# svip-lab/impersonator

Hardware: NVIDIA H100
Metric: frames/sec @256x256 (per-frame inference hot path) (higher is better)
Workload: dtype f16 main product + e4m3 correction products (hi/lo split), f32 accumulate

## Files before the change

### impersonator_b200/csrc/common.cuh

```cuda
#pragma once
#include <cuda_runtime.h>
#include <cuda_fp16.h>
#include <stdint.h>
#include <stdio.h>

#include "../../include/lwb_b200.h"

namespace lwb {

void set_error(const char* fmt, ...);

#define LWB_CHECK_ARG(cond, msg)                                                   \
    do { if (!(cond)) { lwb::set_error("%s: %s", __func__, msg); return LWB_E_INVALID; } } while (0)

#define LWB_CUDA_OK(expr)                                                          \
    do { cudaError_t e__ = (expr); if (e__ != cudaSuccess) {                       \
        lwb::set_error("%s: %s -> %s", __func__, #expr, cudaGetErrorString(e__));  \
        return LWB_E_CUDA; } } while (0)

#define LWB_LAUNCH_OK()                                                            \
    do { cudaError_t e__ = cudaGetLastError(); if (e__ != cudaSuccess) {           \
        lwb::set_error("%s: launch failed -> %s", __func__, cudaGetErrorString(e__)); \
        return LWB_E_CUDA; } } while (0)

static inline int ceil_div(long a, long b) { return (int)((a + b - 1) / b); }

int sm_count();
constexpr int kMaxDevices = 64;
int device_slot();

bool pdl_enabled();
__device__ __forceinline__ void pdl_wait() { asm volatile("griddepcontrol.wait;" ::: "memory"); }
__device__ __forceinline__ void pdl_trigger() { asm volatile("griddepcontrol.launch_dependents;" ::: "memory"); }

template <typename... KArgs, typename... Args>
static inline cudaError_t launch_pdl(void (*kernel)(KArgs...), dim3 grid, dim3 block, size_t smem, cudaStream_t st, Args&&... args)
{
    cudaLaunchConfig_t cfg = {};
    cfg.gridDim = grid; cfg.blockDim = block; cfg.dynamicSmemBytes = smem; cfg.stream = st;
    cudaLaunchAttribute at[1];
    at[0].id = cudaLaunchAttributeProgrammaticStreamSerialization;
    at[0].val.programmaticStreamSerializationAllowed = 1;
    cfg.attrs = at; cfg.numAttrs = pdl_enabled() ? 1 : 0;
    return cudaLaunchKernelEx(&cfg, kernel, static_cast<KArgs>(args)...);
}

__device__ __forceinline__ void ldg_f32x8(const float* p, float* v) {
    const float4 a = __ldg(reinterpret_cast<const float4*>(p)), b = __ldg(reinterpret_cast<const float4*>(p) + 1);
    v[0] = a.x; v[1] = a.y; v[2] = a.z; v[3] = a.w; v[4] = b.x; v[5] = b.y; v[6] = b.z; v[7] = b.w;
}
__device__ __forceinline__ void stg_f32x8(float* p, const float* v) {
    reinterpret_cast<float4*>(p)[0] = make_float4(v[0], v[1], v[2], v[3]);
    reinterpret_cast<float4*>(p)[1] = make_float4(v[4], v[5], v[6], v[7]);
}

}
```

### impersonator_b200/csrc/conv_tc.cu

```cuda
#include <cuda.h>

#include <stdlib.h>

#include <algorithm>
#include <new>
#include <type_traits>

#include "common.cuh"

namespace {

constexpr int TILE_H = 16, TILE_W = 8;
constexpr int SWAP_N_TILE = 64;
constexpr int SWAP_TILE_H = 32;
constexpr int KCHUNK = 64;
constexpr int ROW_BYTES = TILE_W * 128;
constexpr int MAX_TAPS = 49;
constexpr int MAX_GROUP = 8;
constexpr int RING_BYTES = 200 * 1024;
constexpr int MAX_STAGES = 8;
constexpr int NUM_CONSUMERS = 256;
constexpr int NUM_THREADS = NUM_CONSUMERS + 128;
constexpr int MAX_N_TILE = 128;
static_assert(2 * 2 * (TILE_H + MAX_GROUP - 1) * ROW_BYTES + 2 * 2 * MAX_N_TILE * 128 <= RING_BYTES,
// ... 29 lines not shown
struct Cfg {
    static constexpr int B_BYTES = N_TILE * 128;
    static constexpr int B_STAGE_BYTES = B_BYTES * (SPLIT ? 2 : 1);
    static constexpr int BAR_BYTES = 4 * MAX_STAGES * 8;
    static constexpr int STATS_PARTS = N_TILE < SWAP_N_TILE ? 8 : N_TILE == SWAP_N_TILE ? 2 : 0;
    static constexpr int STATS_BYTES = STATS_PARTS * N_TILE * 8;
    static constexpr int SMEM_BYTES = 1024 + RING_BYTES + BAR_BYTES + STATS_BYTES;
    static_assert(B_STAGE_BYTES % 1024 == 0, "B entries must keep the 1024-byte swizzle alignment");
    static_assert(SMEM_BYTES <= 227 * 1024, "exceeds the shared memory of a block");
};

__device__ __forceinline__ uint32_t smem_u32(const void* p) { return (uint32_t)__cvta_generic_to_shared(p); }

__device__ __forceinline__ void mbar_init(uint64_t* bar, uint32_t count) {
    asm volatile("mbarrier.init.shared::cta.b64 [%0], %1;" ::"r"(smem_u32(bar)), "r"(count));
}
__device__ __forceinline__ void mbar_expect_tx(uint64_t* bar, uint32_t bytes) {
    asm volatile("mbarrier.arrive.expect_tx.shared::cta.b64 _, [%0], %1;" ::"r"(smem_u32(bar)), "r"(bytes) : "memory");
}
__device__ __forceinline__ void mbar_arrive(uint64_t* bar) {
    asm volatile("mbarrier.arrive.shared::cta.b64 _, [%0];" ::"r"(smem_u32(bar)) : "memory");
}
__device__ __forceinline__ bool mbar_try_wait(uint64_t* bar, uint32_t parity) {
    uint32_t ok;
    asm volatile("{\n\t.reg .pred p;\n\t"
                 "mbarrier.try_wait.parity.shared::cta.b64 p, [%1], %2;\n\t"
                 "selp.u32 %0, 1, 0, p;\n\t}"
                 : "=r"(ok) : "r"(smem_u32(bar)), "r"(parity) : "memory");
    return ok != 0;
}
__device__ __forceinline__ void mbar_wait(uint64_t* bar, uint32_t parity) {
    if (mbar_try_wait(bar, parity)) return;
    const long long t0 = clock64();
    while (!mbar_try_wait(bar, parity)) {
        if (clock64() - t0 > 4000000000ll) __trap();
    }
}
__device__ __forceinline__ bool elect_one() {
    uint32_t pred;
    asm volatile("{\n\t.reg .pred P;\n\telect.sync _|P, 0xffffffff;\n\tselp.b32 %0, 1, 0, P;\n\t}" : "=r"(pred));
    return pred != 0;
}
__device__ __forceinline__ void fence_barrier_init() { asm volatile("fence.mbarrier_init.release.cluster;" ::: "memory"); }
__device__ __forceinline__ void fence_proxy_async() { asm volatile("fence.proxy.async.shared::cta;" ::: "memory"); }

__device__ __forceinline__ void tma_load_4d(const CUtensorMap* map, void* dst, uint64_t* bar, int c0, int c1, int c2, int c3) {
    asm volatile("cp.async.bulk.tensor.4d.shared::cluster.global.mbarrier::complete_tx::bytes [%0], [%1, {%3, %4, %5, %6}], [%2];"
                 :: "r"(smem_u32(dst)), "l"(map), "r"(smem_u32(bar)), "r"(c0), "r"(c1), "r"(c2), "r"(c3) : "memory");
}
__device__ __forceinline__ void tma_load_3d(const CUtensorMap* map, void* dst, uint64_t* bar, int c0, int c1, int c2) {
    asm volatile("cp.async.bulk.tensor.3d.shared::cluster.global.mbarrier::complete_tx::bytes [%0], [%1, {%3, %4, %5}], [%2];"
                 :: "r"(smem_u32(dst)), "l"(map), "r"(smem_u32(bar)), "r"(c0), "r"(c1), "r"(c2) : "memory");
}

__device__ __forceinline__ uint64_t make_desc(uint32_t smem_addr) {
    return (uint64_t)((smem_addr & 0x3FFFF) >> 4) | (1ull << 16) | (64ull << 32) | (1ull << 62);
}
__device__ __forceinline__ void wgmma_fence() { asm volatile("wgmma.fence.sync.aligned;" ::: "memory"); }
__device__ __forceinline__ void wgmma_commit() { asm volatile("wgmma.commit_group.sync.aligned;" ::: "memory"); }
template <int N>
__device__ __forceinline__ void wgmma_wait() { asm volatile("wgmma.wait_group.sync.aligned %0;" :: "n"(N) : "memory"); }
__device__ __forceinline__ void acc_fence(float& r) { asm volatile("" : "+f"(r) :: "memory"); }

template <int N> __device__ __forceinline__ void wgmma_f16(float* d, uint64_t da, uint64_t db);
template <int N> __device__ __forceinline__ void wgmma_e4m3(float* d, uint64_t da, uint64_t db);
template <> __device__ __forceinline__ void wgmma_f16<16>(float* d, uint64_t da, uint64_t db) {
    asm volatile("{\n\t.reg .pred p;\n\tsetp.ne.b32 p, %10, 0;\n\t"
                 "wgmma.mma_async.sync.aligned.m64n16k16.f32.f16.f16 {%0, %1, %2, %3, %4, %5, %6, %7}, %8, %9, p, 1, 1, 0, 0;\n\t}"
                 : "+f"(d[0]), "+f"(d[1]), "+f"(d[2]), "+f"(d[3]), "+f"(d[4]), "+f"(d[5]), "+f"(d[6]), "+f"(d[7])
                 : "l"(da), "l"(db), "r"(1));
}
template <> __device__ __forceinline__ void wgmma_f16<32>(float* d, uint64_t da, uint64_t db) {
    asm volatile("{\n\t.reg .pred p;\n\tsetp.ne.b32 p, %18, 0;\n\t"
                 "wgmma.mma_async.sync.aligned.m64n32k16.f32.f16.f16 {%0, %1, %2, %3, %4, %5, %6, %7, %8, %9, %10, %11, %12, %13, %14, %15}, %16, %17, p, 1, 1, 0, 0;\n\t}"
                 : "+f"(d[0]), "+f"(d[1]), "+f"(d[2]), "+f"(d[3]), "+f"(d[4]), "+f"(d[5]), "+f"(d[6]), "+f"(d[7]), "+f"(d[8]), "+f"(d[9]), "+f"(d[10]), "+f"(d[11]), "+f"(d[12]), "+f"(d[13]), "+f"(d[14]), "+f"(d[15])
                 : "l"(da), "l"(db), "r"(1));
}
template <> __device__ __forceinline__ void wgmma_f16<128>(float* d, uint64_t da, uint64_t db) {
    asm volatile("{\n\t.reg .pred p;\n\tsetp.ne.b32 p, %66, 0;\n\t"
                 "wgmma.mma_async.sync.aligned.m64n128k16.f32.f16.f16 {%0, %1, %2, %3, %4, %5, %6, %7, %8, %9, %10, %11, %12, %13, %14, %15, %16, %17, %18, %19, %20, %21, %22, %23, %24, %25, %26, %27, %28, %29, %30, %31, %32, %33, %34, %35, %36, %37, %38, %39, %40, %41, %42, %43, %44, %45, %46, %47, %48, %49, %50, %51, %52, %53, %54, %55, %56, %57, %58, %59, %60, %61, %62, %63}, %64, %65, p, 1, 1, 0, 0;\n\t}"
                 : "+f"(d[0]), "+f"(d[1]), "+f"(d[2]), "+f"(d[3]), "+f"(d[4]), "+f"(d[5]), "+f"(d[6]), "+f"(d[7]), "+f"(d[8]), "+f"(d[9]), "+f"(d[10]), "+f"(d[11]), "+f"(d[12]), "+f"(d[13]), "+f"(d[14]), "+f"(d[15]), "+f"(d[16]), "+f"(d[17]), "+f"(d[18]), "+f"(d[19]), "+f"(d[20]), "+f"(d[21]), "+f"(d[22]), "+f"(d[23]), "+f"(d[24]), "+f"(d[25]), "+f"(d[26]), "+f"(d[27]), "+f"(d[28]), "+f"(d[29]), "+f"(d[30]), "+f"(d[31]), "+f"(d[32]), "+f"(d[33]), "+f"(d[34]), "+f"(d[35]), "+f"(d[36]), "+f"(d[37]), "+f"(d[38]), "+f"(d[39]), "+f"(d[40]), "+f"(d[41]), "+f"(d[42]), "+f"(d[43]), "+f"(d[44]), "+f"(d[45]), "+f"(d[46]), "+f"(d[47]), "+f"(d[48]), "+f"(d[49]), "+f"(d[50]), "+f"(d[51]), "+f"(d[52]), "+f"(d[53]), "+f"(d[54]), "+f"(d[55]), "+f"(d[56]), "+f"(d[57]), "+f"(d[58]), "+f"(d[59]), "+f"(d[60]), "+f"(d[61]), "+f"(d[62]), "+f"(d[63])
                 : "l"(da), "l"(db), "r"(1));
}
template <> __device__ __forceinline__ void wgmma_e4m3<16>(float* d, uint64_t da, uint64_t db) {
    asm volatile("{\n\t.reg .pred p;\n\tsetp.ne.b32 p, %10, 0;\n\t"
                 "wgmma.mma_async.sync.aligned.m64n16k32.f32.e4m3.e4m3 {%0, %1, %2, %3, %4, %5, %6, %7}, %8, %9, p, 1, 1;\n\t}"
                 : "+f"(d[0]), "+f"(d[1]), "+f"(d[2]), "+f"(d[3]), "+f"(d[4]), "+f"(d[5]), "+f"(d[6]), "+f"(d[7])
                 : "l"(da), "l"(db), "r"(1));
}
template <> __device__ __forceinline__ void wgmma_e4m3<32>(float* d, uint64_t da, uint64_t db) {
    asm volatile("{\n\t.reg .pred p;\n\tsetp.ne.b32 p, %18, 0;\n\t"
                 "wgmma.mma_async.sync.aligned.m64n32k32.f32.e4m3.e4m3 {%0, %1, %2, %3, %4, %5, %6, %7, %8, %9, %10, %11, %12, %13, %14, %15}, %16, %17, p, 1, 1;\n\t}"
                 : "+f"(d[0]), "+f"(d[1]), "+f"(d[2]), "+f"(d[3]), "+f"(d[4]), "+f"(d[5]), "+f"(d[6]), "+f"(d[7]), "+f"(d[8]), "+f"(d[9]), "+f"(d[10]), "+f"(d[11]), "+f"(d[12]), "+f"(d[13]), "+f"(d[14]), "+f"(d[15])
                 : "l"(da), "l"(db), "r"(1));
}
template <> __device__ __forceinline__ void wgmma_e4m3<128>(float* d, uint64_t da, uint64_t db) {
    asm volatile("{\n\t.reg .pred p;\n\tsetp.ne.b32 p, %66, 0;\n\t"
                 "wgmma.mma_async.sync.aligned.m64n128k32.f32.e4m3.e4m3 {%0, %1, %2, %3, %4, %5, %6, %7, %8, %9, %10, %11, %12, %13, %14, %15, %16, %17, %18, %19, %20, %21, %22, %23, %24, %25, %26, %27, %28, %29, %30, %31, %32, %33, %34, %35, %36, %37, %38, %39, %40, %41, %42, %43, %44, %45, %46, %47, %48, %49, %50, %51, %52, %53, %54, %55, %56, %57, %58, %59, %60, %61, %62, %63}, %64, %65, p, 1, 1;\n\t}"
                 : "+f"(d[0]), "+f"(d[1]), "+f"(d[2]), "+f"(d[3]), "+f"(d[4]), "+f"(d[5]), "+f"(d[6]), "+f"(d[7]), "+f"(d[8]), "+f"(d[9]), "+f"(d[10]), "+f"(d[11]), "+f"(d[12]), "+f"(d[13]), "+f"(d[14]), "+f"(d[15]), "+f"(d[16]), "+f"(d[17]), "+f"(d[18]), "+f"(d[19]), "+f"(d[20]), "+f"(d[21]), "+f"(d[22]), "+f"(d[23]), "+f"(d[24]), "+f"(d[25]), "+f"(d[26]), "+f"(d[27]), "+f"(d[28]), "+f"(d[29]), "+f"(d[30]), "+f"(d[31]), "+f"(d[32]), "+f"(d[33]), "+f"(d[34]), "+f"(d[35]), "+f"(d[36]), "+f"(d[37]), "+f"(d[38]), "+f"(d[39]), "+f"(d[40]), "+f"(d[41]), "+f"(d[42]), "+f"(d[43]), "+f"(d[44]), "+f"(d[45]), "+f"(d[46]), "+f"(d[47]), "+f"(d[48]), "+f"(d[49]), "+f"(d[50]), "+f"(d[51]), "+f"(d[52]), "+f"(d[53]), "+f"(d[54]), "+f"(d[55]), "+f"(d[56]), "+f"(d[57]), "+f"(d[58]), "+f"(d[59]), "+f"(d[60]), "+f"(d[61]), "+f"(d[62]), "+f"(d[63])
                 : "l"(da), "l"(db), "r"(1));
}

__device__ __forceinline__ void consumer_sync() { asm volatile("bar.sync 1, 256;" ::: "memory"); }

struct TileCoord {
    int n_idx, img, y0, x0;
};
template <int TH>
__device__ __forceinline__ TileCoord decode_tile(const ConvParams& P, int tile, int m_tiles) {
    TileCoord t;
    t.n_idx = tile / m_tiles;
    const int m_idx = tile % m_tiles;
    t.img = m_idx / (P.tiles_y * P.tiles_x);
    const int rem = m_idx % (P.tiles_y * P.tiles_x);
    t.y0 = (rem / P.tiles_x) * TH; t.x0 = (rem % P.tiles_x) * TILE_W;
    return t;
}

template <int N_TILE>
__device__ __forceinline__ void warp_tile_stats(const float* acc, bool v0, bool v1, int warp, unsigned lane, float2* s_stats)
{
#pragma unroll
    for (int j = 0; j < N_TILE / 8; j++) {
        const float a0 = v0 ? acc[4 * j] : 0.f, a1 = v0 ? acc[4 * j + 1] : 0.f;
        const float b0 = v1 ? acc[4 * j + 2] : 0.f, b1 = v1 ? acc[4 * j + 3] : 0.f;
        float s0 = a0 + b0, s1 = a1 + b1, q0 = a0 * a0 + b0 * b0, q1 = a1 * a1 + b1 * b1;
#pragma unroll
        for (int off = 4; off <= 16; off <<= 1) {
            s0 += __shfl_xor_sync(0xffffffffu, s0, off); s1 += __shfl_xor_sync(0xffffffffu, s1, off);
            q0 += __shfl_xor_sync(0xffffffffu, q0, off); q1 += __shfl_xor_sync(0xffffffffu, q1, off);
        }
        if (lane < 4) {
            s_stats[warp * N_TILE + 8 * j + 2 * lane] = make_float2(s0, q0);
            s_stats[warp * N_TILE + 8 * j + 2 * lane + 1] = make_float2(s1, q1);
        }
    }
}

template <int N_TILE, int PARTS>
__device__ __forceinline__ void flush_tile_stats(const ConvParams& P, const float2* s_stats, int img, int n_idx)
{
    consumer_sync();
    for (int col = threadIdx.x; col < N_TILE; col += NUM_CONSUMERS) {
        float s = 0.f, q = 0.f;
#pragma unroll
        for (int w = 0; w < PARTS; w++) { const float2 v = s_stats[w * N_TILE + col]; s += v.x; q += v.y; }
        int ch = n_idx * N_TILE + col;
        if (P.phase_cols > 0) ch %= P.phase_cols;
        double* dst = P.stats + 2 * ((size_t)img * P.cout + ch);
        atomicAdd(dst, (double)s);
        atomicAdd(dst + 1, (double)q);
    }
    consumer_sync();
}

template <int N_TILE>
__device__ __forceinline__ void epilogue_plain(const ConvParams& P, float* acc, const TileCoord& t, int warp, unsigned lane,
// ... 74 lines not shown
#pragma unroll
                for (int h = 0; h < 2; h++) {
                    const float a = v ? acc[4 * j + 2 * h + e] : 0.f;
                    s[h] += a; q[h] += a * a;
                }
            }
        }
#pragma unroll
        for (int h = 0; h < 2; h++) {
#pragma unroll
            for (int off = 1; off <= 2; off <<= 1) {
                s[h] += __shfl_xor_sync(0xffffffffu, s[h], off);
                q[h] += __shfl_xor_sync(0xffffffffu, q[h], off);
            }
        }
        if constexpr (N_TILE == SWAP_N_TILE) {
            if ((lane & 3) == 0) {
                s_stats[wg * N_TILE + c0] = make_float2(s[0], q[0]);
                s_stats[wg * N_TILE + c0 + 8] = make_float2(s[1], q[1]);
            }
            flush_tile_stats<N_TILE, 2>(P, s_stats, t.img, t.n_idx);
        } else if ((lane & 3) == 0) {
#pragma unroll
            for (int h = 0; h < 2; h++) {
                double* dst = P.stats + 2 * ((size_t)t.img * P.cout + ch + 8 * h);
                atomicAdd(dst, (double)s[h]);
                atomicAdd(dst + 1, (double)q[h]);
            }
        }
    }
}

enum { MODE_FP16 = 0, MODE_FP16X3 = 1, MODE_F8 = 2 };

template <int N_TILE, int MODE>
struct Regs {
    static constexpr int CONSUMER = N_TILE >= 64 ? (MODE == MODE_F8 ? 168 : 120) : N_TILE == 32 ? 80 : 64;
    static constexpr int LAUNCH = ((2 * CONSUMER + 40 + 2) / 3 + 7) / 8 * 8;
    static constexpr int PRODUCER = 3 * LAUNCH - 2 * CONSUMER;
    static_assert(PRODUCER >= 40 && PRODUCER % 8 == 0 && CONSUMER % 8 == 0, "setmaxnreg takes multiples of 8");
};

template <int N_TILE, bool CM>
__device__ __forceinline__ void mma_f16(float* d, uint64_t act, uint64_t w) {
    if constexpr (CM) wgmma_f16<128>(d, w, act);
    else              wgmma_f16<N_TILE>(d, act, w);
}
template <int N_TILE, bool CM>
__device__ __forceinline__ void mma_e4m3(float* d, uint64_t act, uint64_t w) {
    if constexpr (CM) wgmma_e4m3<128>(d, w, act);
    else              wgmma_e4m3<N_TILE>(d, act, w);
}

template <int N_TILE, int MODE>
__global__ void __launch_bounds__(NUM_THREADS, 1) __maxnreg__((Regs<N_TILE, MODE>::LAUNCH))
k_conv_wg(const __grid_constant__ ConvParams P)
{
    constexpr bool CM = N_TILE >= SWAP_N_TILE;
    constexpr bool SPLIT = MODE != MODE_FP16;
    constexpr int TH = N_TILE == SWAP_N_TILE ? SWAP_TILE_H : TILE_H;
    constexpr int ACC = CM ? 64 : N_TILE / 2;
    using C = Cfg<N_TILE, SPLIT>;
    extern __shared__ uint8_t smem_raw[];
    uint8_t* smem = reinterpret_cast<uint8_t*>((reinterpret_cast<uintptr_t>(smem_raw) + 1023) & ~(uintptr_t)1023);
    const int a_op_bytes = P.a_rows * ROW_BYTES;
    const int a_stage_bytes = a_op_bytes * (SPLIT ? 2 : 1);
    uint8_t* b_ring = smem + P.a_stages * a_stage_bytes;
    uint64_t* a_full = reinterpret_cast<uint64_t*>(smem + RING_BYTES);
    uint64_t* a_empty = a_full + MAX_STAGES;
    uint64_t* b_full = a_empty + MAX_STAGES;
    uint64_t* b_empty = b_full + MAX_STAGES;
    float2* s_stats = reinterpret_cast<float2*>(smem + RING_BYTES + C::BAR_BYTES);

    const int warp = threadIdx.x >> 5;
    const unsigned lane = threadIdx.x & 31;

    if (threadIdx.x == 0) {
        for (int s = 0; s < P.a_stages; s++) { mbar_init(a_full + s, 1); mbar_init(a_empty + s, NUM_CONSUMERS / 32); }
        for (int s = 0; s < P.b_stages; s++) { mbar_init(b_full + s, 1); mbar_init(b_empty + s, NUM_CONSUMERS / 32); }
        fence_barrier_init();
        fence_proxy_async();
    }
    __syncthreads();
    lwb::pdl_wait();
    lwb::pdl_trigger();

    const int nchunks = P.chunks0 + P.chunks1;
    const int m_tiles = P.n_img * P.tiles_y * P.tiles_x;
    const int total = m_tiles * P.n_tiles_n;

    if (warp >= NUM_CONSUMERS / 32) {
        asm volatile("setmaxnreg.dec.sync.aligned.u32 %0;" :: "n"(Regs<N_TILE, MODE>::PRODUCER));
        if (warp != NUM_CONSUMERS / 32) return;
        if (elect_one()) {
            asm volatile("prefetch.tensormap [%0];" :: "l"(&P.a_hi[0]) : "memory");
            asm volatile("prefetch.tensormap [%0];" :: "l"(&P.w_hi) : "memory");
            if (SPLIT) {
                asm volatile("prefetch.tensormap [%0];" :: "l"(&P.a_lo[0]) : "memory");
                asm volatile("prefetch.tensormap [%0];" :: "l"(&P.w_lo) : "memory");
            }
        }
        int as = 0, bs = 0; uint32_t aph = 0, bph = 0;
        for (int tile = blockIdx.x; tile < total; tile += gridDim.x) {
            const TileCoord t = decode_tile<TH>(P, tile, m_tiles);
            for (int g = 0; g < P.ngroups; g++) {
                const int first = P.g_first[g], cnt = P.g_cnt[g];
                const int xx = t.x0 + P.dx[first], yy = t.y0 + P.dy[first];
                for (int chunk = 0; chunk < nchunks; chunk++) {
                    const bool second = chunk >= P.chunks0;
                    const int mi = second ? 1 : P.tmap[first];
                    const int c0 = (second ? chunk - P.chunks0 : chunk) * KCHUNK;
                    mbar_wait(a_empty + as, aph ^ 1);
                    uint8_t* sa = smem + as * a_stage_bytes;
                    if (elect_one()) {
                        mbar_expect_tx(a_full + as, (uint32_t)a_stage_bytes);
                        tma_load_4d(&P.a_hi[mi], sa, a_full + as, c0, xx, yy, t.img);
                        if (SPLIT) tma_load_4d(&P.a_lo[mi], sa + a_op_bytes, a_full + as, c0, xx, yy, t.img);
                    }
                    __syncwarp();
                    if (++as == P.a_stages) { as = 0; aph ^= 1; }
                    for (int i = 0; i < cnt; i++) {
                        mbar_wait(b_empty + bs, bph ^ 1);
                        uint8_t* sb = b_ring + bs * C::B_STAGE_BYTES;
                        const int wt = P.wtap[first + i];
                        if (elect_one()) {
                            mbar_expect_tx(b_full + bs, (uint32_t)C::B_STAGE_BYTES);
                            tma_load_3d(&P.w_hi, sb, b_full + bs, chunk * KCHUNK, t.n_idx * N_TILE, wt);
                            if (SPLIT) tma_load_3d(&P.w_lo, sb + C::B_BYTES, b_full + bs, chunk * KCHUNK, t.n_idx * N_TILE, wt);
                        }
                        __syncwarp();
                        if (++bs == P.b_stages) { bs = 0; bph ^= 1; }
                    }
                }
            }
        }
    } else {
        asm volatile("setmaxnreg.inc.sync.aligned.u32 %0;" :: "n"(Regs<N_TILE, MODE>::CONSUMER));
        constexpr bool CH_SPLIT = N_TILE == MAX_N_TILE;
        const uint32_t wg = (uint32_t)(warp >> 2);
        const uint32_t a_base = smem_u32(smem) + (CH_SPLIT ? 0 : wg * (TH / 2) * ROW_BYTES);
        const uint32_t b_base = smem_u32(b_ring) + (CH_SPLIT ? wg * 64 * 128 : 0);
        float acc[ACC];
        float acc8[MODE == MODE_F8 ? ACC : 1];
        int as = 0, bs = 0; uint32_t aph = 0, bph = 0;
        for (int tile = blockIdx.x; tile < total; tile += gridDim.x) {
            const TileCoord t = decode_tile<TH>(P, tile, m_tiles);
#pragma unroll
            for (int i = 0; i < ACC; i++) acc[i] = 0.f;
#pragma unroll
            for (int i = 0; i < (MODE == MODE_F8 ? ACC : 1); i++) acc8[i] = 0.f;
            int prev_b = -1, prev_a = -1;
            for (int g = 0; g < P.ngroups; g++) {
                const int cnt = P.g_cnt[g];
                for (int chunk = 0; chunk < nchunks; chunk++) {
                    mbar_wait(a_full + as, aph);
                    const uint32_t a_hi = a_base + as * a_stage_bytes;
                    for (int i = 0; i < cnt; i++) {
                        mbar_wait(b_full + bs, bph);
                        const uint32_t ai = a_hi + i * ROW_BYTES, al = ai + a_op_bytes;
                        const uint32_t b_hi = b_base + bs * C::B_STAGE_BYTES, b_lo = b_hi + C::B_BYTES;
                        wgmma_fence();
#pragma unroll
                        for (int k = 0; k < KCHUNK / 16; k++) {
                            const uint64_t da = make_desc(ai + k * 32), db = make_desc(b_hi + k * 32);
                            mma_f16<N_TILE, CM>(acc, da, db);
                            if constexpr (MODE == MODE_F8) {
                                mma_e4m3<N_TILE, CM>(acc8, make_desc(al + k * 32), make_desc(b_lo + k * 32));
                            } else if constexpr (MODE == MODE_FP16X3) {
                                mma_f16<N_TILE, CM>(acc, da, make_desc(b_lo + k * 32));
                                mma_f16<N_TILE, CM>(acc, make_desc(al + k * 32), db);
                            }
                        }
                        wgmma_commit();
                        if (prev_b >= 0) {
                            wgmma_wait<1>();
                            if (lane == 0) {
                                mbar_arrive(b_empty + prev_b);
                                if (prev_a >= 0) mbar_arrive(a_empty + prev_a);
                            }
                            prev_a = -1;
                        }
                        prev_b = bs;
                        if (++bs == P.b_stages) { bs = 0; bph ^= 1; }
                    }
                    prev_a = as;
                    if (++as == P.a_stages) { as = 0; aph ^= 1; }
                }
            }
            wgmma_wait<0>();
#pragma unroll
            for (int i = 0; i < ACC; i++) acc_fence(acc[i]);
            if constexpr (MODE == MODE_F8) {
#pragma unroll
                for (int i = 0; i < ACC; i++) { acc_fence(acc8[i]); acc[i] += acc8[i]; }
            }
            if (lane == 0) { mbar_arrive(b_empty + prev_b); mbar_arrive(a_empty + prev_a); }
            if constexpr (CM) epilogue_channel_major<N_TILE>(P, acc, t, warp, lane, s_stats);
            else              epilogue_plain<N_TILE>(P, acc, t, warp, lane, s_stats);
        }
    }
}

typedef CUresult (*EncodeTiledFn)(CUtensorMap*, CUtensorMapDataType, cuuint32_t, void*, const cuuint64_t*,
                                  const cuuint64_t*, const cuuint32_t*, const cuuint32_t*, CUtensorMapInterleave,
                                  CUtensorMapSwizzle, CUtensorMapL2promotion, CUtensorMapFloatOOBfill);

EncodeTiledFn get_encode()
{
    static EncodeTiledFn fn = nullptr;
    if (!fn) {
        void* p = nullptr;
        cudaDriverEntryPointQueryResult q;
        if (cudaGetDriverEntryPoint("cuTensorMapEncodeTiled", &p, cudaEnableDefault, &q) != cudaSuccess || !p) return nullptr;
        fn = (EncodeTiledFn)p;
    }
    return fn;
}

int encode_map(CUtensorMap* m, const void* base, int rank, const uint64_t* dims, const uint64_t* strides_bytes, const uint32_t* box)
{
    EncodeTiledFn enc = get_encode();
    if (!enc) { lwb::set_error("cuTensorMapEncodeTiled entry point not available"); return LWB_E_CUDA; }
    cuuint64_t gdim[5]; cuuint64_t gstr[4]; cuuint32_t bx[5]; cuuint32_t es[5];
    for (int i = 0; i < rank; i++) { gdim[i] = dims[i]; bx[i] = box[i]; es[i] = 1; }
    for (int i = 0; i < rank - 1; i++) gstr[i] = strides_bytes[i];
    CUresult r = enc(m, CU_TENSOR_MAP_DATA_TYPE_FLOAT16, (cuuint32_t)rank, const_cast<void*>(base), gdim, gstr, bx, es,
                     CU_TENSOR_MAP_INTERLEAVE_NONE, CU_TENSOR_MAP_SWIZZLE_128B, CU_TENSOR_MAP_L2_PROMOTION_L2_256B,
                     CU_TENSOR_MAP_FLOAT_OOB_FILL_NONE);
    if (r != CUDA_SUCCESS) {
        lwb::set_error("cuTensorMapEncodeTiled failed (%d): rank %d dims [%llu,%llu,%llu,%llu] strides [%llu,%llu,%llu] box [%u,%u,%u,%u]",
                       (int)r, rank, (unsigned long long)dims[0], (unsigned long long)dims[1], (unsigned long long)(rank > 2 ? dims[2] : 0),
                       (unsigned long long)(rank > 3 ? dims[3] : 0), (unsigned long long)strides_bytes[0],
                       (unsigned long long)(rank > 2 ? strides_bytes[1] : 0), (unsigned long long)(rank > 3 ? strides_bytes[2] : 0),
                       box[0], box[1], rank > 2 ? box[2] : 0, rank > 3 ? box[3] : 0);
        return LWB_E_CUDA;
    }
    return LWB_OK;
}

struct Launch {
    ConvParams p;
    int n_tile;
    int mode;
    int grid;
};

template <int N_TILE, int MODE>
int launch_wg(const Launch& L, cudaStream_t st)
{
    using C = Cfg<N_TILE, MODE != MODE_FP16>;
    static bool attr_set_dev[lwb::kMaxDevices] = {};
    bool& attr_set = attr_set_dev[lwb::device_slot()];
    if (!attr_set) {
        LWB_CUDA_OK(cudaFuncSetAttribute(k_conv_wg<N_TILE, MODE>, cudaFuncAttributeMaxDynamicSharedMemorySize, C::SMEM_BYTES));
        attr_set = true;
    }
    LWB_CUDA_OK(lwb::launch_pdl(k_conv_wg<N_TILE, MODE>, dim3(L.grid), dim3(NUM_THREADS), C::SMEM_BYTES, st, L.p));
    LWB_LAUNCH_OK();
    return LWB_OK;
}

template <class F>
int with_instance(int n_tile, int mode, F&& f)
{
    auto modes = [&](auto nt) {
        if (mode == MODE_F8) return f(nt, std::integral_constant<int, MODE_F8>());
        if (mode == MODE_FP16X3) return f(nt, std::integral_constant<int, MODE_FP16X3>());
        return f(nt, std::integral_constant<int, MODE_FP16>());
    };
    switch (n_tile) {
        case 16:  return modes(std::integral_constant<int, 16>());
        case 32:  return modes(std::integral_constant<int, 32>());
        case 64:  return modes(std::integral_constant<int, 64>());
        case 128: return modes(std::integral_constant<int, 128>());
    }
    lwb::set_error("conv_tc: unsupported N tile %d", n_tile);
    return LWB_E_UNSUPPORTED;
}

int launch(const Launch& L, cudaStream_t st)
{
    return with_instance(L.n_tile, L.mode,
                         [&](auto nt, auto md) { return launch_wg<decltype(nt)::value, decltype(md)::value>(L, st); });
}

int pick_n_tile(int cout, int forced)
{
    if (forced > 0) return forced > MAX_N_TILE && forced % MAX_N_TILE == 0 ? MAX_N_TILE : forced;
    if (cout % 128 == 0) return 128;
    if (cout % 64 == 0) return 64;
    if (cout % 32 == 0) return 32;
    if (cout % 16 == 0) return 16;
    return -1;
}

struct View {
    const uint16_t* hi;
    const uint16_t* lo;
    uint64_t dims[4], str[3];
};

struct LaunchSpec {
    int ntaps;
    signed char dy[MAX_TAPS], dx[MAX_TAPS], tmap[MAX_TAPS];
    short wtap[MAX_TAPS];
    int chunks0, chunks1;
    int nviews;
    View a[4];
    View w;
    int ncols;
    int dom_h, dom_w;
    int oy_mul, oy_add, ox_mul, ox_add, phase_cols;
    int n_tile;

    void tap(int y, int x, int view, int wt)
    {
        dy[ntaps] = (signed char)y; dx[ntaps] = (signed char)x; tmap[ntaps] = (signed char)view; wtap[ntaps] = (short)wt;
        ntaps++;
    }
};

}

struct lwb_conv_plan {
    int num;
    Launch launches[4];
};

static bool rowk_cin(int cin0) { return cin0 == 8 || cin0 == 16 || cin0 == 24; }

static View nhwc_view(const uint16_t* hi, const uint16_t* lo, int n, int h, int w, int c, int step = 1, int py = 0, int px = 0)
{
    const size_t off = ((size_t)py * w + px) * c;
    return View{hi + off, lo ? lo + off : lo,
                {(uint64_t)c, (uint64_t)((w - px + step - 1) / step), (uint64_t)((h - py + step - 1) / step), (uint64_t)n},
                {(uint64_t)step * c * 2, (uint64_t)step * w * c * 2, (uint64_t)h * w * c * 2}};
}

static View weight_view(const uint16_t* hi, const uint16_t* lo, int k, int ncols, int taps)
{
    return View{hi, lo, {(uint64_t)k, (uint64_t)ncols, (uint64_t)taps}, {(uint64_t)k * 2, (uint64_t)ncols * k * 2}};
}

static int encode_pair(CUtensorMap* hi, CUtensorMap* lo, int rank, const View& v, const uint32_t* box, bool split)
{
    const int rc = encode_map(hi, v.hi, rank, v.dims, v.str, box);
    return rc != LWB_OK || !split ? rc : encode_map(lo, v.lo, rank, v.dims, v.str, box);
}

static void group_taps(ConvParams& p, int tile_h)
{
    int order[MAX_TAPS];
    for (int t = 0; t < p.ntaps; t++) order[t] = t;
    std::stable_sort(order, order + p.ntaps, [&](int a, int b) {
        if (p.tmap[a] != p.tmap[b]) return p.tmap[a] < p.tmap[b];
        if (p.dx[a] != p.dx[b]) return p.dx[a] < p.dx[b];
        return p.dy[a] < p.dy[b];
    });
    const ConvParams src = p;
    int longest = 0;
    p.ngroups = 0;
    for (int t = 0; t < p.ntaps; t++) {
        const int o = order[t];
        p.dy[t] = src.dy[o]; p.dx[t] = src.dx[o]; p.tmap[t] = src.tmap[o]; p.wtap[t] = src.wtap[o];
        const bool joins = t > 0 && p.tmap[t] == p.tmap[t - 1] && p.dx[t] == p.dx[t - 1] && p.dy[t] == p.dy[t - 1] + 1 &&
                           p.g_cnt[p.ngroups - 1] < MAX_GROUP;
        if (!joins) { p.g_first[p.ngroups] = (signed char)t; p.g_cnt[p.ngroups] = 0; p.ngroups++; }
        p.g_cnt[p.ngroups - 1]++;
        longest = std::max(longest, (int)p.g_cnt[p.ngroups - 1]);
    }
    p.a_rows = tile_h + longest - 1;
}

static void pick_rings(ConvParams& p, int n_tile, bool split)
{
    const int ops = split ? 2 : 1;
    const int a_bytes = p.a_rows * ROW_BYTES * ops, b_bytes = n_tile * 128 * ops;
    const int longest = p.a_rows - tile_rows(n_tile) + 1;
    int best = 0;
    for (int a = 2; a <= MAX_STAGES; a++) {
        const int b = std::min(MAX_STAGES, (RING_BYTES - a * a_bytes) / b_bytes);
        if (b < 2) break;
        if (std::min(a * longest, b) > best) { best = std::min(a * longest, b); p.a_stages = a; p.b_stages = b; }
    }
}

static int build_launch(Launch& L, const LaunchSpec& s, const lwb_conv_desc* d, float* out_raw, double* stats, int sms)
{
    const bool split = d->split != 0;
    ConvParams& p = L.p;
    memset(&p, 0, sizeof(p));
    p.ntaps = s.ntaps; p.chunks0 = s.chunks0; p.chunks1 = s.chunks1;
    for (int t = 0; t < s.ntaps; t++) { p.dy[t] = s.dy[t]; p.dx[t] = s.dx[t]; p.tmap[t] = s.tmap[t]; p.wtap[t] = s.wtap[t]; }
    group_taps(p, tile_rows(s.n_tile));
    int rc;
    const uint32_t a_box[4] = {KCHUNK, TILE_W, (uint32_t)p.a_rows, 1};
    for (int v = 0; v < s.nviews; v++)
        if ((rc = encode_pair(&p.a_hi[v], &p.a_lo[v], 4, s.a[v], a_box, split)) != LWB_OK) return rc;
    const uint32_t w_box[3] = {KCHUNK, (uint32_t)s.n_tile, 1};
    if ((rc = encode_pair(&p.w_hi, &p.w_lo, 3, s.w, w_box, split)) != LWB_OK) return rc;
    p.n_img = d->n;
    p.dom_h = s.dom_h; p.dom_w = s.dom_w;
    p.tiles_y = lwb::ceil_div(s.dom_h, tile_rows(s.n_tile)); p.tiles_x = lwb::ceil_div(s.dom_w, TILE_W);
    p.n_tiles_n = s.ncols / s.n_tile;
    p.out = out_raw; p.out_h = d->h_out; p.out_w = d->w_out; p.cout = d->cout;
    p.oy_mul = s.oy_mul; p.oy_add = s.oy_add; p.ox_mul = s.ox_mul; p.ox_add = s.ox_add; p.phase_cols = s.phase_cols;
    p.stats = stats;
    p.out_scale = ldexpf(1.f, -d->w_exp);
    L.n_tile = s.n_tile; L.mode = d->split;
    pick_rings(p, s.n_tile, split);
    const long total = (long)p.n_img * p.tiles_y * p.tiles_x * p.n_tiles_n;
    L.grid = (int)(total < sms ? total : sms);
    return LWB_OK;
}

extern "C" int lwb_conv_plan_create(const lwb_conv_desc* d,
                                    const uint16_t* x0_hi, const uint16_t* x0_lo,
                                    const uint16_t* x1_hi, const uint16_t* x1_lo,
                                    const uint16_t* w_hi, const uint16_t* w_lo,
                                    float* out_raw, double* stats, lwb_conv_plan** plan_out)
{
    LWB_CHECK_ARG(d && x0_hi && w_hi && out_raw && plan_out, "null pointer");
    const bool split = d->split != 0;
    const bool f8 = d->split == 2;
    LWB_CHECK_ARG(d->split >= 0 && d->split <= 2, "split must be 0, 1 or 2");
    LWB_CHECK_ARG(!split || (x0_lo && w_lo), "split mode needs the lo operands");
    LWB_CHECK_ARG(!f8 || (!d->rowk && !d->halo), "the fp8 lo mode is not available for row-K / halo plans");
    LWB_CHECK_ARG(d->n > 0 && d->h_in > 0 && d->w_in > 0 && d->cout > 0, "non-positive size");
    LWB_CHECK_ARG(d->cout % 16 == 0, "cout must be a multiple of 16");
    LWB_CHECK_ARG(d->w_exp >= -40 && d->w_exp <= 60, "w_exp out of range");
    const int n_tile = pick_n_tile(d->cout, d->n_tile);
    LWB_CHECK_ARG(n_tile > 0 && d->cout % n_tile == 0, "no N tile divides cout");
    if (d->halo) {
        LWB_CHECK_ARG(d->stride == 1 && !d->transposed && d->dil == 1, "halo mode needs stride 1, dilation 1, not transposed");
        if (d->rowk) LWB_CHECK_ARG(d->kw <= 8 && rowk_cin(d->cin0) && d->cin1 == 0 && d->row_pitch >= d->w_in + 8, "row-K shape");
        else         LWB_CHECK_ARG(d->kw <= 9 && (d->kw & 1) && (d->kh & 1), "halo mode needs an odd kernel, kw <= 9, with 'same' padding (kh/2, kw/2)");
    }

    const int sms = lwb::sm_count();

    LaunchSpec s = {};
    s.n_tile = n_tile; s.ncols = d->cout;
    s.dom_h = d->h_out; s.dom_w = d->w_out;
    s.oy_mul = s.ox_mul = 1;
    s.nviews = 1;
    LaunchSpec specs[4];
    int num = 1;
    if (d->rowk) {
        LWB_CHECK_ARG(d->stride == 1 && !d->transposed && d->kw <= 8, "row-K needs stride 1, kw <= 8, 8 channels");
        LWB_CHECK_ARG(rowk_cin(d->cin0) && d->cin1 == 0, "row-K needs 8, 16 or 24 padded input channels in one input");
        LWB_CHECK_ARG(d->h_out == d->h_in && d->w_out == d->w_in && d->row_pitch >= d->w_in + 8, "row-K shape");
        for (int ky = 0; ky < d->kh; ky++) s.tap(ky, 0, 0, ky);
        const int k_row = 8 * d->cin0;
        s.chunks0 = k_row / KCHUNK;
        const uint64_t hp = d->h_in + d->kh - 1, px_bytes = (uint64_t)d->cin0 * 2, row_bytes = (uint64_t)d->row_pitch * px_bytes;
        s.a[0] = View{x0_hi, x0_lo, {(uint64_t)k_row, (uint64_t)d->w_in, hp, (uint64_t)d->n}, {px_bytes, row_bytes, hp * row_bytes}};
        s.w = weight_view(w_hi, w_lo, k_row, d->cout, d->kh);
    } else {
        LWB_CHECK_ARG(d->cin0 % KCHUNK == 0 && d->cin1 % KCHUNK == 0 && d->cin0 > 0, "input channels must be multiples of 64");
        LWB_CHECK_ARG(d->cin1 == 0 || (x1_hi && (!split || x1_lo)), "second input missing");
        const int cin_total = d->cin0 + d->cin1;
        const int ntaps_w = d->kh * d->kw;
        LWB_CHECK_ARG(ntaps_w <= MAX_TAPS, "too many filter taps");
        s.chunks0 = d->cin0 / KCHUNK; s.chunks1 = d->cin1 / KCHUNK;
        s.a[0] = nhwc_view(x0_hi, x0_lo, d->n, d->h_in, d->w_in, d->cin0);
// ... 38 lines not shown
                s.a[1] = nhwc_view(x1_hi, x1_lo, d->n, d->h_in, d->w_in, d->cin1);
            }
        }
    }
    if (num == 1) specs[0] = s;

    lwb_conv_plan* plan = new (std::nothrow) lwb_conv_plan();
    LWB_CHECK_ARG(plan, "out of host memory");
    for (; plan->num < num; plan->num++) {
        const int rc = build_launch(plan->launches[plan->num], specs[plan->num], d, out_raw, stats, sms);
        if (rc != LWB_OK) { delete plan; return rc; }
    }
    *plan_out = plan;
    return LWB_OK;
}

extern "C" int lwb_conv_plan_run(const lwb_conv_plan* plan, lwb_stream_t stream)
{
    LWB_CHECK_ARG(plan, "null plan");
    for (int i = 0; i < plan->num; i++) {
        const int rc = launch(plan->launches[i], (cudaStream_t)stream);
        if (rc != LWB_OK) return rc;
    }
    return LWB_OK;
}

extern "C" void lwb_conv_plan_destroy(lwb_conv_plan* plan) { delete plan; }

extern "C" int lwb_conv_plan_num_launches(const lwb_conv_plan* plan) { return plan ? plan->num : 0; }

extern "C" int lwb_conv_plan_launch_info(const lwb_conv_plan* plan, int i, int* out)
{
    LWB_CHECK_ARG(plan && out, "null pointer");
    LWB_CHECK_ARG(i >= 0 && i < plan->num, "launch index out of range");
    const Launch& L = plan->launches[i];
    out[0] = L.n_tile; out[1] = L.mode; out[2] = L.p.chunks0 + L.p.chunks1; out[3] = L.p.ntaps;
    return LWB_OK;
}

extern "C" int lwb_conv2d_nhwc(const lwb_conv_desc* d,
                               const uint16_t* x0_hi, const uint16_t* x0_lo,
                               const uint16_t* x1_hi, const uint16_t* x1_lo,
                               const uint16_t* w_hi, const uint16_t* w_lo,
                               float* out_raw, double* stats, lwb_stream_t stream)
{
    lwb_conv_plan* plan = nullptr;
    int rc = lwb_conv_plan_create(d, x0_hi, x0_lo, x1_hi, x1_lo, w_hi, w_lo, out_raw, stats, &plan);
    if (rc != LWB_OK) return rc;
    rc = lwb_conv_plan_run(plan, stream);
    lwb_conv_plan_destroy(plan);
    return rc;
}

template <int N_TILE, int MODE>
static int conv_resources(int* out)
{
    using C = Cfg<N_TILE, MODE != MODE_FP16>;
    cudaFuncAttributes a;
    LWB_CUDA_OK(cudaFuncSetAttribute(k_conv_wg<N_TILE, MODE>, cudaFuncAttributeMaxDynamicSharedMemorySize, C::SMEM_BYTES));
    LWB_CUDA_OK(cudaFuncGetAttributes(&a, k_conv_wg<N_TILE, MODE>));
    int blocks = 0;
    LWB_CUDA_OK(cudaOccupancyMaxActiveBlocksPerMultiprocessor(&blocks, k_conv_wg<N_TILE, MODE>, NUM_THREADS, C::SMEM_BYTES));
    out[0] = a.numRegs; out[1] = (int)a.sharedSizeBytes; out[2] = C::SMEM_BYTES; out[3] = (int)a.localSizeBytes;
    out[4] = NUM_THREADS; out[5] = blocks; out[6] = Regs<N_TILE, MODE>::CONSUMER;
    return LWB_OK;
}

extern "C" int lwb_conv_kernel_resources(int n_tile, int mode, int* out)
{
    LWB_CHECK_ARG(out, "null pointer");
    LWB_CHECK_ARG(mode >= 0 && mode <= 2, "mode must be 0, 1 or 2");
    return with_instance(n_tile, mode,
                         [&](auto nt, auto md) { return conv_resources<decltype(nt)::value, decltype(md)::value>(out); });
}
```

Measured before the change: 2338.

## Pair CTAs in 2-wide clusters and multicast weight tiles via TMA

```diff
diff --git a/impersonator_b200/csrc/common.cuh b/impersonator_b200/csrc/common.cuh
--- a/impersonator_b200/csrc/common.cuh
+++ b/impersonator_b200/csrc/common.cuh
@@ -34,15 +34,28 @@
 __device__ __forceinline__ void pdl_trigger() { asm volatile("griddepcontrol.launch_dependents;" ::: "memory"); }
 
 template <typename... KArgs, typename... Args>
-static inline cudaError_t launch_pdl(void (*kernel)(KArgs...), dim3 grid, dim3 block, size_t smem, cudaStream_t st, Args&&... args)
+static inline cudaError_t launch_pdl_cluster(void (*kernel)(KArgs...), dim3 grid, dim3 block, size_t smem, cudaStream_t st,
+                                             int cluster_x, Args&&... args)
 {
     cudaLaunchConfig_t cfg = {};
     cfg.gridDim = grid; cfg.blockDim = block; cfg.dynamicSmemBytes = smem; cfg.stream = st;
-    cudaLaunchAttribute at[1];
-    at[0].id = cudaLaunchAttributeProgrammaticStreamSerialization;
-    at[0].val.programmaticStreamSerializationAllowed = 1;
-    cfg.attrs = at; cfg.numAttrs = pdl_enabled() ? 1 : 0;
+    cudaLaunchAttribute at[2];
+    int n = 0;
+    if (pdl_enabled()) {
+        at[n].id = cudaLaunchAttributeProgrammaticStreamSerialization;
+        at[n++].val.programmaticStreamSerializationAllowed = 1;
+    }
+    if (cluster_x > 1) {
+        at[n].id = cudaLaunchAttributeClusterDimension;
+        at[n++].val.clusterDim = {(unsigned)cluster_x, 1, 1};
+    }
+    cfg.attrs = at; cfg.numAttrs = n;
     return cudaLaunchKernelEx(&cfg, kernel, static_cast<KArgs>(args)...);
+}
+template <typename... KArgs, typename... Args>
+static inline cudaError_t launch_pdl(void (*kernel)(KArgs...), dim3 grid, dim3 block, size_t smem, cudaStream_t st, Args&&... args)
+{
+    return launch_pdl_cluster(kernel, grid, block, smem, st, 1, static_cast<Args&&>(args)...);
 }
 
 __device__ __forceinline__ void ldg_f32x8(const float* p, float* v) {
diff --git a/impersonator_b200/csrc/conv_tc.cu b/impersonator_b200/csrc/conv_tc.cu
--- a/impersonator_b200/csrc/conv_tc.cu
+++ b/impersonator_b200/csrc/conv_tc.cu
@@ -105,6 +105,25 @@
     asm volatile("cp.async.bulk.tensor.3d.shared::cluster.global.mbarrier::complete_tx::bytes [%0], [%1, {%3, %4, %5}], [%2];"
                  :: "r"(smem_u32(dst)), "l"(map), "r"(smem_u32(bar)), "r"(c0), "r"(c1), "r"(c2) : "memory");
 }
+__device__ __forceinline__ void tma_load_3d_multicast(const CUtensorMap* map, void* dst, uint64_t* bar, int c0, int c1, int c2,
+                                                      uint16_t mask) {
+    asm volatile("cp.async.bulk.tensor.3d.shared::cluster.global.mbarrier::complete_tx::bytes.multicast::cluster [%0], [%1, {%3, %4, %5}], [%2], %6;"
+                 :: "r"(smem_u32(dst)), "l"(map), "r"(smem_u32(bar)), "r"(c0), "r"(c1), "r"(c2), "h"(mask) : "memory");
+}
+
+__device__ __forceinline__ uint32_t cluster_ctarank() {
+    uint32_t r;
+    asm volatile("mov.u32 %0, %%cluster_ctarank;" : "=r"(r));
+    return r;
+}
+__device__ __forceinline__ void cluster_sync() {
+    asm volatile("barrier.cluster.arrive.release;\n\tbarrier.cluster.wait.acquire;" ::: "memory");
+}
+__device__ __forceinline__ void mbar_arrive_remote(uint64_t* bar, uint32_t rank) {
+    asm volatile("{\n\t.reg .b32 ra;\n\tmapa.shared::cluster.u32 ra, %0, %1;\n\t"
+                 "mbarrier.arrive.shared::cluster.b64 _, [ra];\n\t}"
+                 :: "r"(smem_u32(bar)), "r"(rank) : "memory");
+}
 
 __device__ __forceinline__ uint64_t make_desc(uint32_t smem_addr) {
     return (uint64_t)((smem_addr & 0x3FFFF) >> 4) | (1ull << 16) | (64ull << 32) | (1ull << 62);
@@ -156,6 +175,13 @@
 
 __device__ __forceinline__ void consumer_sync() { asm volatile("bar.sync 1, 256;" ::: "memory"); }
 
+template <bool PAIR>
+__device__ __forceinline__ int unit_tile(int u, int mp, int m_tiles, uint32_t rank, bool& own) {
+    if (!PAIR) { own = true; return u; }
+    const int m = 2 * (u % mp) + (int)rank;
+    own = m < m_tiles;
+    return (u / mp) * m_tiles + (own ? m : m - 1);
+}
 struct TileCoord {
     int n_idx, img, y0, x0;
 };
@@ -336,10 +362,11 @@
     else              wgmma_e4m3<N_TILE>(d, act, w);
 }
 
-template <int N_TILE, int MODE>
+template <int N_TILE, int MODE, bool PAIR>
 __global__ void __launch_bounds__(NUM_THREADS, 1) __maxnreg__((Regs<N_TILE, MODE>::LAUNCH))
 k_conv_wg(const __grid_constant__ ConvParams P)
 {
+    static_assert(!PAIR || N_TILE == MAX_N_TILE, "CTA pairs split the weight rows of a 128-wide N tile");
     constexpr bool CM = N_TILE >= SWAP_N_TILE;
     constexpr bool SPLIT = MODE != MODE_FP16;
     constexpr int TH = N_TILE == SWAP_N_TILE ? SWAP_TILE_H : TILE_H;
@@ -361,17 +388,21 @@
 
     if (threadIdx.x == 0) {
         for (int s = 0; s < P.a_stages; s++) { mbar_init(a_full + s, 1); mbar_init(a_empty + s, NUM_CONSUMERS / 32); }
-        for (int s = 0; s < P.b_stages; s++) { mbar_init(b_full + s, 1); mbar_init(b_empty + s, NUM_CONSUMERS / 32); }
+        for (int s = 0; s < P.b_stages; s++) { mbar_init(b_full + s, 1); mbar_init(b_empty + s, (PAIR ? 2 : 1) * NUM_CONSUMERS / 32); }
         fence_barrier_init();
         fence_proxy_async();
     }
-    __syncthreads();
+    if constexpr (PAIR) cluster_sync();
+    else                __syncthreads();
     lwb::pdl_wait();
     lwb::pdl_trigger();
 
     const int nchunks = P.chunks0 + P.chunks1;
     const int m_tiles = P.n_img * P.tiles_y * P.tiles_x;
-    const int total = m_tiles * P.n_tiles_n;
+    const uint32_t rank = PAIR ? cluster_ctarank() : 0;
+    const int mp = PAIR ? (m_tiles + 1) / 2 : m_tiles;
+    const int units = mp * P.n_tiles_n;
+    const int u0 = PAIR ? (int)(blockIdx.x >> 1) : (int)blockIdx.x, stride = PAIR ? (int)(gridDim.x >> 1) : (int)gridDim.x;
 
     if (warp >= NUM_CONSUMERS / 32) {
         asm volatile("setmaxnreg.dec.sync.aligned.u32 %0;" :: "n"(Regs<N_TILE, MODE>::PRODUCER));
@@ -385,8 +416,9 @@
             }
         }
         int as = 0, bs = 0; uint32_t aph = 0, bph = 0;
-        for (int tile = blockIdx.x; tile < total; tile += gridDim.x) {
-            const TileCoord t = decode_tile<TH>(P, tile, m_tiles);
+        for (int u = u0; u < units; u += stride) {
+            bool own;
+            const TileCoord t = decode_tile<TH>(P, unit_tile<PAIR>(u, mp, m_tiles, rank, own), m_tiles);
             for (int g = 0; g < P.ngroups; g++) {
                 const int first = P.g_first[g], cnt = P.g_cnt[g];
                 const int xx = t.x0 + P.dx[first], yy = t.y0 + P.dy[first];
@@ -409,8 +441,15 @@
                         const int wt = P.wtap[first + i];
                         if (elect_one()) {
                             mbar_expect_tx(b_full + bs, (uint32_t)C::B_STAGE_BYTES);
-                            tma_load_3d(&P.w_hi, sb, b_full + bs, chunk * KCHUNK, t.n_idx * N_TILE, wt);
-                            if (SPLIT) tma_load_3d(&P.w_lo, sb + C::B_BYTES, b_full + bs, chunk * KCHUNK, t.n_idx * N_TILE, wt);
+                            if constexpr (PAIR) {
+                                const int row = 64 * (int)rank;
+                                tma_load_3d_multicast(&P.w_hi, sb + row * 128, b_full + bs, chunk * KCHUNK, t.n_idx * N_TILE + row, wt, 0x3);
+                                if (SPLIT) tma_load_3d_multicast(&P.w_lo, sb + C::B_BYTES + row * 128, b_full + bs, chunk * KCHUNK,
+                                                                 t.n_idx * N_TILE + row, wt, 0x3);
+                            } else {
+                                tma_load_3d(&P.w_hi, sb, b_full + bs, chunk * KCHUNK, t.n_idx * N_TILE, wt);
+                                if (SPLIT) tma_load_3d(&P.w_lo, sb + C::B_BYTES, b_full + bs, chunk * KCHUNK, t.n_idx * N_TILE, wt);
+                            }
                         }
                         __syncwarp();
                         if (++bs == P.b_stages) { bs = 0; bph ^= 1; }
@@ -426,9 +465,14 @@
         const uint32_t b_base = smem_u32(b_ring) + (CH_SPLIT ? wg * 64 * 128 : 0);
         float acc[ACC];
         float acc8[MODE == MODE_F8 ? ACC : 1];
+        auto release_b = [&](int s) {
+            mbar_arrive(b_empty + s);
+            if constexpr (PAIR) mbar_arrive_remote(b_empty + s, rank ^ 1);
+        };
         int as = 0, bs = 0; uint32_t aph = 0, bph = 0;
-        for (int tile = blockIdx.x; tile < total; tile += gridDim.x) {
-            const TileCoord t = decode_tile<TH>(P, tile, m_tiles);
+        for (int u = u0; u < units; u += stride) {
+            bool own;
+            const TileCoord t = decode_tile<TH>(P, unit_tile<PAIR>(u, mp, m_tiles, rank, own), m_tiles);
 #pragma unroll
             for (int i = 0; i < ACC; i++) acc[i] = 0.f;
 #pragma unroll
@@ -459,7 +503,7 @@
                         if (prev_b >= 0) {
                             wgmma_wait<1>();
                             if (lane == 0) {
-                                mbar_arrive(b_empty + prev_b);
+                                release_b(prev_b);
                                 if (prev_a >= 0) mbar_arrive(a_empty + prev_a);
                             }
                             prev_a = -1;
@@ -478,11 +522,13 @@
 #pragma unroll
                 for (int i = 0; i < ACC; i++) { acc_fence(acc8[i]); acc[i] += acc8[i]; }
             }
-            if (lane == 0) { mbar_arrive(b_empty + prev_b); mbar_arrive(a_empty + prev_a); }
+            if (lane == 0) { release_b(prev_b); mbar_arrive(a_empty + prev_a); }
+            if (!own) continue;
             if constexpr (CM) epilogue_channel_major<N_TILE>(P, acc, t, warp, lane, s_stats);
             else              epilogue_plain<N_TILE>(P, acc, t, warp, lane, s_stats);
         }
     }
+    if constexpr (PAIR) cluster_sync();
 }
 
 typedef CUresult (*EncodeTiledFn)(CUtensorMap*, CUtensorMapDataType, cuuint32_t, void*, const cuuint64_t*,
@@ -526,37 +572,54 @@
     ConvParams p;
     int n_tile;
     int mode;
+    bool pair;
     int grid;
 };
 
-template <int N_TILE, int MODE>
-int launch_wg(const Launch& L, cudaStream_t st)
-{
-    using C = Cfg<N_TILE, MODE != MODE_FP16>;
+template <int N_TILE, int MODE, bool PAIR>
+int set_smem_attr()
+{
     static bool attr_set_dev[lwb::kMaxDevices] = {};
     bool& attr_set = attr_set_dev[lwb::device_slot()];
     if (!attr_set) {
-        LWB_CUDA_OK(cudaFuncSetAttribute(k_conv_wg<N_TILE, MODE>, cudaFuncAttributeMaxDynamicSharedMemorySize, C::SMEM_BYTES));
+        LWB_CUDA_OK(cudaFuncSetAttribute(k_conv_wg<N_TILE, MODE, PAIR>, cudaFuncAttributeMaxDynamicSharedMemorySize,
+                                         Cfg<N_TILE, MODE != MODE_FP16>::SMEM_BYTES));
         attr_set = true;
     }
-    LWB_CUDA_OK(lwb::launch_pdl(k_conv_wg<N_TILE, MODE>, dim3(L.grid), dim3(NUM_THREADS), C::SMEM_BYTES, st, L.p));
+    return LWB_OK;
+}
+
+template <int N_TILE, int MODE, bool PAIR>
+int launch_wg(const Launch& L, cudaStream_t st)
+{
+    using C = Cfg<N_TILE, MODE != MODE_FP16>;
+    const int rc = set_smem_attr<N_TILE, MODE, PAIR>();
+    if (rc != LWB_OK) return rc;
+    LWB_CUDA_OK(lwb::launch_pdl_cluster(k_conv_wg<N_TILE, MODE, PAIR>, dim3(L.grid), dim3(NUM_THREADS), C::SMEM_BYTES, st,
+                                        PAIR ? 2 : 1, L.p));
     LWB_LAUNCH_OK();
     return LWB_OK;
 }
 
 template <class F>
-int with_instance(int n_tile, int mode, F&& f)
-{
-    auto modes = [&](auto nt) {
-        if (mode == MODE_F8) return f(nt, std::integral_constant<int, MODE_F8>());
-        if (mode == MODE_FP16X3) return f(nt, std::integral_constant<int, MODE_FP16X3>());
-        return f(nt, std::integral_constant<int, MODE_FP16>());
+int with_instance(int n_tile, int mode, bool pair, F&& f)
+{
+    auto modes = [&](auto nt, auto pr) {
+        if (mode == MODE_F8) return f(nt, std::integral_constant<int, MODE_F8>(), pr);
+        if (mode == MODE_FP16X3) return f(nt, std::integral_constant<int, MODE_FP16X3>(), pr);
+        return f(nt, std::integral_constant<int, MODE_FP16>(), pr);
     };
+    const std::false_type single;
+    if (pair && n_tile != MAX_N_TILE) {
+        lwb::set_error("conv_tc: CTA pairs need an N tile of %d, not %d", MAX_N_TILE, n_tile);
+        return LWB_E_UNSUPPORTED;
+    }
     switch (n_tile) {
-        case 16:  return modes(std::integral_constant<int, 16>());
-        case 32:  return modes(std::integral_constant<int, 32>());
-        case 64:  return modes(std::integral_constant<int, 64>());
-        case 128: return modes(std::integral_constant<int, 128>());
+        case 16:  return modes(std::integral_constant<int, 16>(), single);
+        case 32:  return modes(std::integral_constant<int, 32>(), single);
+        case 64:  return modes(std::integral_constant<int, 64>(), single);
+        case 128: return pair ? modes(std::integral_constant<int, 128>(), std::true_type())
+                              : modes(std::integral_constant<int, 128>(), single);
     }
     lwb::set_error("conv_tc: unsupported N tile %d", n_tile);
     return LWB_E_UNSUPPORTED;
@@ -564,8 +627,32 @@
 
 int launch(const Launch& L, cudaStream_t st)
 {
-    return with_instance(L.n_tile, L.mode,
-                         [&](auto nt, auto md) { return launch_wg<decltype(nt)::value, decltype(md)::value>(L, st); });
+    return with_instance(L.n_tile, L.mode, L.pair, [&](auto nt, auto md, auto pr) {
+        return launch_wg<decltype(nt)::value, decltype(md)::value, decltype(pr)::value>(L, st);
+    });
+}
+
+int max_active_pairs(int mode)
+{
+    static int pairs_dev[lwb::kMaxDevices][3] = {};
+    int& pairs = pairs_dev[lwb::device_slot()][mode];
+    if (pairs == 0) {
+        int rc = with_instance(MAX_N_TILE, mode, true, [&](auto nt, auto md, auto pr) {
+            constexpr int N = decltype(nt)::value, M = decltype(md)::value;
+            const int r = set_smem_attr<N, M, decltype(pr)::value>();
+            if (r != LWB_OK) return r;
+            cudaLaunchConfig_t cfg = {};
+            cfg.gridDim = dim3(2 * lwb::sm_count()); cfg.blockDim = dim3(NUM_THREADS);
+            cfg.dynamicSmemBytes = Cfg<N, M != MODE_FP16>::SMEM_BYTES;
+            cudaLaunchAttribute at;
+            at.id = cudaLaunchAttributeClusterDimension; at.val.clusterDim = {2, 1, 1};
+            cfg.attrs = &at; cfg.numAttrs = 1;
+            LWB_CUDA_OK(cudaOccupancyMaxActiveClusters(&pairs, k_conv_wg<N, M, decltype(pr)::value>, &cfg));
+            return LWB_OK;
+        });
+        if (rc != LWB_OK) return -1;
+    }
+    return pairs;
 }
 
 int pick_n_tile(int cout, int forced)
@@ -669,6 +756,8 @@
     }
 }
 
+constexpr int PAIR_MIN_K_STEPS = 16;
+
 static int build_launch(Launch& L, const LaunchSpec& s, const lwb_conv_desc* d, float* out_raw, double* stats, int sms)
 {
     const bool split = d->split != 0;
@@ -677,11 +766,12 @@
     p.ntaps = s.ntaps; p.chunks0 = s.chunks0; p.chunks1 = s.chunks1;
     for (int t = 0; t < s.ntaps; t++) { p.dy[t] = s.dy[t]; p.dx[t] = s.dx[t]; p.tmap[t] = s.tmap[t]; p.wtap[t] = s.wtap[t]; }
     group_taps(p, tile_rows(s.n_tile));
+    L.pair = s.n_tile == MAX_N_TILE && s.ntaps * (s.chunks0 + s.chunks1) >= PAIR_MIN_K_STEPS;
     int rc;
     const uint32_t a_box[4] = {KCHUNK, TILE_W, (uint32_t)p.a_rows, 1};
     for (int v = 0; v < s.nviews; v++)
         if ((rc = encode_pair(&p.a_hi[v], &p.a_lo[v], 4, s.a[v], a_box, split)) != LWB_OK) return rc;
-    const uint32_t w_box[3] = {KCHUNK, (uint32_t)s.n_tile, 1};
+    const uint32_t w_box[3] = {KCHUNK, (uint32_t)(L.pair ? s.n_tile / 2 : s.n_tile), 1};
     if ((rc = encode_pair(&p.w_hi, &p.w_lo, 3, s.w, w_box, split)) != LWB_OK) return rc;
     p.n_img = d->n;
     p.dom_h = s.dom_h; p.dom_w = s.dom_w;
@@ -693,8 +783,19 @@
     p.out_scale = ldexpf(1.f, -d->w_exp);
     L.n_tile = s.n_tile; L.mode = d->split;
     pick_rings(p, s.n_tile, split);
-    const long total = (long)p.n_img * p.tiles_y * p.tiles_x * p.n_tiles_n;
-    L.grid = (int)(total < sms ? total : sms);
+    const long m_tiles = (long)p.n_img * p.tiles_y * p.tiles_x;
+    if (L.pair) {
+        const int resident = max_active_pairs(d->split);
+        if (resident <= 0) {
+            if (resident == 0) lwb::set_error("conv_tc: no CTA pair of the N = %d instance fits on this device", MAX_N_TILE);
+            return resident == 0 ? LWB_E_UNSUPPORTED : LWB_E_CUDA;
+        }
+        const long pairs = std::min<long>((m_tiles + 1) / 2 * p.n_tiles_n, sms / 2);
+        L.grid = 2 * (int)pairs;
+    } else {
+        const long total = m_tiles * p.n_tiles_n;
+        L.grid = (int)(total < sms ? total : sms);
+    }
     return LWB_OK;
 }
 
@@ -839,15 +940,15 @@
     return rc;
 }
 
-template <int N_TILE, int MODE>
+template <int N_TILE, int MODE, bool PAIR>
 static int conv_resources(int* out)
 {
     using C = Cfg<N_TILE, MODE != MODE_FP16>;
     cudaFuncAttributes a;
-    LWB_CUDA_OK(cudaFuncSetAttribute(k_conv_wg<N_TILE, MODE>, cudaFuncAttributeMaxDynamicSharedMemorySize, C::SMEM_BYTES));
-    LWB_CUDA_OK(cudaFuncGetAttributes(&a, k_conv_wg<N_TILE, MODE>));
+    LWB_CUDA_OK(cudaFuncSetAttribute(k_conv_wg<N_TILE, MODE, PAIR>, cudaFuncAttributeMaxDynamicSharedMemorySize, C::SMEM_BYTES));
+    LWB_CUDA_OK(cudaFuncGetAttributes(&a, k_conv_wg<N_TILE, MODE, PAIR>));
     int blocks = 0;
-    LWB_CUDA_OK(cudaOccupancyMaxActiveBlocksPerMultiprocessor(&blocks, k_conv_wg<N_TILE, MODE>, NUM_THREADS, C::SMEM_BYTES));
+    LWB_CUDA_OK(cudaOccupancyMaxActiveBlocksPerMultiprocessor(&blocks, k_conv_wg<N_TILE, MODE, PAIR>, NUM_THREADS, C::SMEM_BYTES));
     out[0] = a.numRegs; out[1] = (int)a.sharedSizeBytes; out[2] = C::SMEM_BYTES; out[3] = (int)a.localSizeBytes;
     out[4] = NUM_THREADS; out[5] = blocks; out[6] = Regs<N_TILE, MODE>::CONSUMER;
     return LWB_OK;
@@ -857,6 +958,7 @@
 {
     LWB_CHECK_ARG(out, "null pointer");
     LWB_CHECK_ARG(mode >= 0 && mode <= 2, "mode must be 0, 1 or 2");
-    return with_instance(n_tile, mode,
-                         [&](auto nt, auto md) { return conv_resources<decltype(nt)::value, decltype(md)::value>(out); });
-}
+    return with_instance(n_tile, mode, n_tile == MAX_N_TILE, [&](auto nt, auto md, auto pr) {
+        return conv_resources<decltype(nt)::value, decltype(md)::value, decltype(pr)::value>(out);
+    });
+}
```

Measured after the change: 2346, median of 6. About the same (+0.3%).
